# getzlab/rnaseqc

Hardware: AMD Instinct MI355X
Metric: reads/sec whole-node (100 M-read synthetic BAM, GENCODE GTF) at 1/2/4/8 GPU -- `value`: the hot path over the records resident in HBM (the bench contract's definition of value); `whole_node.value`: the same job from the BAM file to the reports (CLI `Average Reads/Sec` window), checked against `value (higher is better)
Workload: dtype i32/u64 counters, f64 exon fractions

## Files before the change

rnaseqc_amd/csrc/rsqc_api.cpp:

```cpp
#include "rsqc_ctx.h"
#include "rsqc_index.h"

namespace rsqc {

int fail(rsqc_ctx *c, int code, const std::string &msg) {
    if (c) { c->last_error = msg; }
    return code;
}
int dev_alloc(rsqc_ctx *c, DevBuf &b, size_t bytes, bool zero) {
    if (bytes == 0) bytes = 16;
    bytes = (bytes + 15) & ~(size_t)15;
    if (b.bytes < bytes) {
        b.release();
        HIP_TRY(c, hipMalloc(&b.p, bytes));
        b.bytes = bytes;
    }
    if (zero) HIP_TRY(c, hipMemsetAsync(b.p, 0, b.bytes, c->stream));
    return 0;
}

static int zero_accumulators(rsqc_ctx *c) {
    launch_reset(c->stream, c->d_arena.p, c->arena_bytes, c->d_cov.p, c->d_cov.bytes, (uint32_t *)((char *)c->d_arena.p + c->off_misc + 36));
    HIP_TRY(c, hipGetLastError());
    for (auto &pb : c->pair_pool) pb.used = false;
    c->pairs_in_flight.clear();
    c->pair_arena.used = c->frag_arena.used = c->gc_arena.used = 0;
    for (auto &fb : c->frag_pool) fb.used = false;
    c->frags_in_flight.clear();
    c->h_fsize.clear(); c->h_fcount.clear();
    c->frag_remaining = c->have_bed ? c->params.fragment_samples : 0;
    for (auto &gb : c->gc_pool) gb.used = false;
    c->gcs_in_flight.clear();
    if (c->have_ref) {
        HIP_TRY(c, hipMemsetAsync(c->d_gc_bins.p, 0, (RSQC_GC_BINS + 1) * 8, c->stream));
        c->h_gc.assign(RSQC_GC_BINS + 1, 0);
    }
    c->finalized = false;
// ... 27 lines not shown
        delete c;
        return RSQC_ERR_HIP;
    }
    c->dparams.mapq_threshold = params->mapq_threshold;
    c->dparams.base_mismatch = params->base_mismatch;
    c->dparams.chimeric_distance = params->chimeric_distance;
    c->dparams.stranded = params->stranded;
    c->dparams.unpaired = params->unpaired;
    c->dparams.exclude_chimeric = params->exclude_chimeric;
    c->dparams.n_filter_tags = params->n_filter_tags;
    c->dparams.legacy = params->legacy ? 1 : 0;
    c->pair_arena.n_col = 1; c->pair_arena.width[0] = sizeof(PairRec);
    c->frag_arena.n_col = 6; { const size_t w[6] = {8, 8, 4, 4, 4, 4}; for (int k = 0; k < 6; ++k) c->frag_arena.width[k] = w[k]; }
    c->gc_arena.n_col = 7; { const size_t w[7] = {8, 8, 4, 4, 4, 4, 4}; for (int k = 0; k < 7; ++k) c->gc_arena.width[k] = w[k]; }
    if (const char *e = getenv("RSQC_K1_GRID")) c->k1_grid = std::min(16384, std::max(1, atoi(e)));
    *out = c;
    return RSQC_OK;
}

void rsqc_destroy(rsqc_ctx *c) {
    if (!c) return;
    (void)hipSetDevice(c->device);
    (void)hipStreamSynchronize(c->stream);
    for (auto *u : c->resident) if (u) free_batch(u);
    for (auto *u : c->transient) free_batch(u);
    for (auto &b : c->upload_pool) b.release();
    for (auto &b : c->ann_bufs) b.release();
    for (auto &pb : c->pair_pool) { pb.rec.release(); pb.counts.release(); if (pb.h_counts) (void)hipHostFree(pb.h_counts); if (pb.done) (void)hipEventDestroy(pb.done); if (pb.kernels) (void)hipEventDestroy(pb.kernels); }
    for (auto &fb : c->frag_pool) { fb.file.release(); fb.qhash.release(); fb.name.release(); fb.endpos.release(); fb.fs.release(); fb.h2.release(); fb.count.release(); fb.r_file.release(); fb.r_qhash.release(); fb.r_name.release(); fb.r_endpos.release(); fb.r_fs.release(); fb.r_h2.release(); fb.r_counts.release(); if (fb.h_count) (void)hipHostFree(fb.h_count); }
    for (auto &gb : c->gc_pool) { gb.file.release(); gb.qhash.release(); gb.row.release(); gb.endpos.release(); gb.flag_lq.release(); gb.tid.release(); gb.h2.release(); gb.count.release(); if (gb.h_count) (void)hipHostFree(gb.h_count); }
// ... 15 lines not shown
    track_drop(c, true);
    for (auto &b : c->parked) b.release();
    free_sort_scratch(c->gc_scratch); free_sort_scratch(c->frag_scratch);
    c->d_ref_bits.release(); c->d_ref_off.release(); c->d_ref_len.release(); c->d_gc_bins.release(); c->d_exon_gc.release();
    DevBuf *all[] = {&c->d_arena, &c->d_cov, &c->d_ovf_index, &c->d_tiles, &c->d_defer, &c->d_ei_rank, &c->d_table, &c->d_tab_off, &c->d_tab_cap};
    if (c->h_arena) (void)hipHostFree(c->h_arena);
    if (c->h_rl_raw) (void)hipHostFree(c->h_rl_raw);
    if (c->stream2) (void)hipStreamDestroy(c->stream2);
    if (c->stream3) (void)hipStreamDestroy(c->stream3);
    if (c->stream4) (void)hipStreamDestroy(c->stream4);
    if (c->ev_join3) (void)hipEventDestroy(c->ev_join3);
    if (c->ev_join4) (void)hipEventDestroy(c->ev_join4);
    if (c->ev_fork) (void)hipEventDestroy(c->ev_fork);
    if (c->ev_retired) (void)hipEventDestroy(c->ev_retired);
    if (c->ev_join) (void)hipEventDestroy(c->ev_join);
    for (auto *b : all) b->release();
    for (auto &pr : c->k1_events) { (void)hipEventDestroy(pr.first); (void)hipEventDestroy(pr.second); }
    for (auto &pr : c->long_events) (void)hipEventDestroy(pr.second);
    for (auto e : c->event_pool) (void)hipEventDestroy(e);
    (void)hipStreamDestroy(c->stream);
    delete c;
}

int rsqc_set_annotation(rsqc_ctx *c, const rsqc_annotation *a, const uint8_t *owned_contig) {
    if (!c || !a) return RSQC_ERR_ARG;
    if (c->have_ann) return fail(c, RSQC_ERR_ARG, "annotation already set");
    HIP_TRY(c, hipSetDevice(c->device));
    const int nc = a->n_contigs, G = a->n_genes, L = a->n_genes_listed, E = a->n_exons;
    c->n_ref = a->n_ref; c->n_contigs = nc; c->n_genes = G; c->n_listed = L; c->n_exons = E;
    HostIndex hx;
// ... 65 lines not shown
    c->off_gcv = at; at += Lz * 8;
    c->off_ecv = at; at += Ez * 8;
    c->off_gvalid = at; at += pad8(Lz);
    c->off_ecvv = at; at += pad8(Ez);
    c->off_ehit = at; at += pad8(Ez);
    at = (at + 15) & ~(size_t)15;
    c->off_misc = at; at += 64;
    c->arena_bytes = at;
    if ((rc = dev_alloc(c, c->d_arena, at, false))) return rc;
    HIP_TRY(c, hipHostMalloc((void **)&c->h_arena, at, hipHostMallocDefault));
    if ((rc = dev_alloc(c, c->d_cov, (size_t)(run + 64) * 4, false))) return rc;
    const uint32_t ovf_cap = 1u << 20;
    if ((rc = dev_alloc(c, c->d_ovf_index, (size_t)ovf_cap * 8, false))) return rc;
    for (hipStream_t *s : {&c->stream2, &c->stream3, &c->stream4})
        if (!*s) HIP_TRY(c, hipStreamCreateWithPriority(s, hipStreamNonBlocking, c->prio_side));
    for (hipEvent_t *e : {&c->ev_join3, &c->ev_join4, &c->ev_fork, &c->ev_join, &c->ev_retired})
        if (!*e) HIP_TRY(c, hipEventCreateWithFlags(e, hipEventDisableTiming));
    char *A = (char *)c->d_arena.p;
    DevAccum &acc = c->acc;
    acc.gene_reads = (unsigned long long *)(A + c->off_u64);
    acc.gene_unique = acc.gene_reads + G;
    acc.gene_frag = acc.gene_unique + G;
    acc.counters = acc.gene_frag + G;
    acc.exon_acc = (double *)(A + c->off_exon);
    acc.cov_diff = (uint32_t *)c->d_cov.p;
    acc.ovf_count = (uint32_t *)(A + c->off_misc);
    acc.read_length = (int32_t *)(A + c->off_misc + 8);
    acc.error = (int *)(A + c->off_misc + 16);
    acc.rl_stats = (uint32_t *)(A + c->off_misc + 32);
    acc.defer_total = (uint32_t *)(A + c->off_misc + 48);
    acc.ovf_index = (uint64_t *)c->d_ovf_index.p; acc.ovf_cap = ovf_cap;
    c->have_ann = true;
    if ((rc = zero_accumulators(c))) return rc;
    HIP_TRY(c, hipStreamSynchronize(c->stream));
    c->last_error = hx.warning;
    c->n_exons_outside_gene = hx.n_exons_outside_gene;
    return RSQC_OK;
}

int rsqc_set_reference(rsqc_ctx *c, const rsqc_reference *ref) {
    if (!c || !ref || !c->have_ann) return RSQC_ERR_ARG;
    if (c->have_ref) return fail(c, RSQC_ERR_ARG, "reference already set");
    HIP_TRY(c, hipSetDevice(c->device));
    const int nc = c->n_contigs;
    std::vector<unsigned long long> off((size_t)nc, ~0ull), len((size_t)nc, 0ull);
    unsigned long long words = 0, longest = 0;
    for (int i = 0; i < ref->n; ++i) {
// ... 124 lines not shown
    c->arena_bytes = 0;
    c->dann = DevAnnotation{}; c->dref = DevReference{};
    uint32_t *const tile_span = c->acc.tile_span;
    c->acc = DevAccum{}; c->acc.tile_span = tile_span;
    c->d_ge_off = c->d_ge_row = c->d_gene_cov_off = c->d_gene_coding = c->d_gene_order = nullptr;
    c->d_gene_flags = c->d_gene_owned = nullptr;
    c->n_ref = c->n_contigs = c->n_genes = c->n_listed = c->n_exons = 0;
    c->k3_large = c->k3_medium = c->k3_xlarge = c->k3_le6144 = c->k3_le3072 = c->k3_le2048 = c->k3_le1024 = 0;
    c->cov_entries = 0; c->n_exons_outside_gene = 0;
    std::vector<uint32_t>().swap(c->exon_row_id);
    std::vector<double>().swap(c->h_exon_gc);
    c->h_gc.clear();
    c->have_ann = c->have_bed = c->have_ref = false;
    free_sort_scratch(c->gc_scratch); free_sort_scratch(c->frag_scratch);
    c->h_fsize.clear(); c->h_fcount.clear(); c->frag_remaining = 0; c->frag_kept = 0;
    c->finalized = false; c->early_copied = false;
    c->next_record_base = 0; c->name_mode = -1; c->have_ranges = false; c->have_composed_rl = false;
    c->batch_file_index.clear(); c->batch_records.clear();
    c->h_rl_offset.clear(); c->h_rl_span.clear(); c->h_rl_state.clear();
    c->h_sample_file.clear(); c->h_sample_size.clear();
    c->results = rsqc_results{};
    c->sticky = 0;
    c->last_error.clear();
    return RSQC_OK;
}

void *rsqc_host_alloc(size_t bytes) {
    void *p = nullptr;
    if (hipHostMalloc(&p, bytes ? bytes : 16, hipHostMallocDefault) != hipSuccess) { (void)hipGetLastError(); return nullptr; }
    return p;
}
// ... 49 lines not shown
```

rnaseqc_amd/csrc/rsqc_ctx.h:

```cpp
#pragma once
#include <algorithm>
#include <chrono>
#include <cstdio>
#include <cstdlib>
#include <cstring>
#include <string>
#include <vector>

#include "rsqc_device.h"
#include "rsqc_decode.h"
#include "rsqc_sam.h"

#if defined(RSQC_K1_PROF) || defined(RSQC_DIAG_KNOBS)
#define RSQC_DIAG(name) getenv(name)
namespace rsqc {
inline void host_trace(const char *what) {
    static const bool on = getenv("RSQC_HOST_TRACE") != nullptr;
    if (!on) return;
    static std::chrono::steady_clock::time_point last = std::chrono::steady_clock::now();
    const auto now = std::chrono::steady_clock::now();
    fprintf(stderr, "[host] %-28s +%8.1f us\n", what, std::chrono::duration<double, std::micro>(now - last).count());
    last = now;
}
}
// ... 145 lines not shown
    uint32_t k3_large = 0, k3_medium = 0, k3_xlarge = 0, k3_le6144 = 0, k3_le3072 = 0, k3_le2048 = 0, k3_le1024 = 0;
    int stream_prio = 0, prio_side = 0;
    uint32_t n_exons_outside_gene = 0;
    hipEvent_t fin_e0 = nullptr, fin_e1 = nullptr;
    uint64_t cov_entries = 0;
    bool have_bed = false;

    DevBuf d_arena, d_cov, d_ovf_index, d_tiles;
    DevBuf d_defer;
    DevBuf d_ei_rank;
    char *h_arena = nullptr;
    size_t arena_bytes = 0, off_u64 = 0, off_exon = 0, off_gmean = 0, off_gstd = 0, off_gcv = 0, off_bias3 = 0,
           off_bias5 = 0, off_ecv = 0, off_gvalid = 0, off_ecvv = 0, off_ehit = 0, off_misc = 0;
    hipStream_t stream2 = nullptr, stream3 = nullptr, stream4 = nullptr;
    hipEvent_t ev_fork = nullptr, ev_join = nullptr, ev_join3 = nullptr, ev_join4 = nullptr, ev_retired = nullptr;
    DevAccum acc{};
    uint64_t tile_cap = 0;
    std::vector<PairBuf> pair_pool;
    std::vector<size_t> pairs_in_flight;
    Arena pair_arena, frag_arena, gc_arena;
    DevBuf d_arena_count;
    std::vector<DevBuf> parked;
    DevBuf d_table, d_tab_off, d_tab_cap;
    std::vector<FragBuf> frag_pool;
    std::vector<size_t> frags_in_flight;
    uint32_t frag_remaining = 0;
    bool have_ref = false;
    DevBuf d_ref_bits, d_ref_off, d_ref_len, d_gc_bins, d_exon_gc;
    DevReference dref{};
    std::vector<GcBuf> gc_pool;
    std::vector<size_t> gcs_in_flight;
    std::vector<uint64_t> h_gc;
    std::vector<double> h_exon_gc;
    SortScratch gc_scratch, frag_scratch;
    uint32_t frag_kept = 0;
    bool finalized = false;

    std::vector<UploadedBatch *> resident;
// ... 75 lines not shown
```

rnaseqc_amd/csrc/rsqc_device.h:

```cpp
#pragma once

#if !defined(RSQC_WAVE_EMU)
#include <hip/hip_runtime.h>
#endif
#include <stdint.h>

#include "rsqc_read.h"

#define RSQC_K1_THREADS 256
#define RSQC_MAX_BIAS_WINDOW 1024
#define RSQC_K3_THREADS 1024
#include "rsqc_k3_plan.h"

namespace rsqc {

struct DevBatch {
    uint64_t n;
    uint64_t record_base;
    const rsqc_rec_core *core;
    const rsqc_rec_aux *aux;
    const uint32_t *cigar;
    const uint32_t *qhash2;
    uint32_t n_seg;
    const int32_t *seg_tid;
// ... 86 lines not shown
    const unsigned long long *gene_reads;
    uint32_t *cov;
    int32_t n_listed;
    uint32_t mask; int32_t bias_offset, bias_window; uint64_t bias_gene_length;
    double *g_mean, *g_std, *g_cv; uint8_t *g_valid;
    double *e_cv; uint8_t *e_cv_valid;
    unsigned long long *bias3, *bias5;
    int *error;
};
void launch_gene_coverage(hipStream_t s, hipStream_t s2, hipStream_t s3, const GeneCovArgs &A, uint32_t n_large, uint32_t n_medium, uint32_t n_xlarge,
                          uint32_t n_le6144 = 0, uint32_t n_le3072 = 0, uint32_t n_le2048 = 0, uint32_t n_le1024 = 0);

void launch_reduce_add(hipStream_t s, unsigned long long *du, const unsigned long long *su, size_t nu, double *df, const double *sf, size_t nf,
                       uint8_t *db, const uint8_t *sb, size_t nb);
void launch_pack_results(hipStream_t s, const double *exon_acc, uint8_t *exon_hit, uint32_t n_exons);
void launch_reset(hipStream_t s, void *arena, size_t arena_bytes, void *cov, size_t cov_bytes, uint32_t *rl_min);
void launch_classify(hipStream_t s, int grid, int variant, const DevAnnotation &a, const DevParams &p, const DevBatch &b,
                     const DevAccum &acc);
inline int rsqc_long_grid(int k1_grid) { return k1_grid < 1024 ? k1_grid : 1024; }
void launch_classify_long(hipStream_t s, int k1_grid, const DevAnnotation &a, const DevParams &p, const DevBatch &b, const DevAccum &acc);
void launch_ei_rank(hipStream_t s, const EiEntry *ei, uint32_t ei_lo, uint32_t ei_hi, EiRank *rank, uint32_t n_words);
void launch_classify_slow(hipStream_t s, const DevAnnotation &a, const DevParams &p, const DevBatch &b,
                          const DevAccum &acc);
#define RSQC_RL_SUMMARY_WORDS (2 + 2 * 128)
void launch_read_length(hipStream_t s, const DevAnnotation &a, const DevParams &p, const DevBatch &b,
                        const DevAccum &acc, uint32_t *summary);
#define RSQC_SLOW_RES 2048u
#define RSQC_SLOW_LEGACY_GRID 4096u
#ifndef RSQC_K4_PART_READS
#define RSQC_K4_PART_READS 1024
#endif
#define RSQC_K4_SUB_CAP (2 * RSQC_K4_PART_READS)
#define RSQC_K4_PART_SLOTS (4 * RSQC_K4_PART_READS)
#ifndef RSQC_K4_COUNT_THREADS
#define RSQC_K4_COUNT_THREADS 256
#endif
struct FragKey { uint32_t lo, hi, h2; };
struct FragPlan {
    uint32_t *part_first;
    uint32_t *cursor;
    uint4 *ginfo;
    uint4 *part_info;
    uint32_t *full_list, *full_n;
    FragKey *list;
    unsigned long long *blk_space; uint32_t *blk_parts;
};
void launch_frag_layout(hipStream_t s, const unsigned long long *gene_reads, uint32_t n_genes, const FragPlan &P, int *error);
void launch_frag_local(hipStream_t s, const DevAccum &acc, uint32_t n_chunks, const FragPlan &P, uint32_t list_blocks);
void launch_pairs_append(hipStream_t s, const PairRec *src, uint32_t chunk_cap, const uint32_t *counts,
                         uint32_t n_chunks, uint32_t slow_base, uint32_t slow_cap, PairRec *dst);
void launch_frag_count(hipStream_t s, uint32_t n_genes, const FragPlan &P, uint32_t parts_bound, unsigned long long *gene_frag, int *error);

}

#include <vector>
namespace rsqc {
struct SortScratch { void *k0 = nullptr, *k1 = nullptr, *v0 = nullptr, *v1 = nullptr, *v2 = nullptr, *v3 = nullptr, *tmp = nullptr, *count = nullptr;
                     size_t cap_n = 0, tmp_bytes = 0; uint32_t *table = nullptr, *out_size = nullptr, *out_count = nullptr; };
void free_sort_scratch(SortScratch &s);
int run_fragment_sizes(hipStream_t stream, const FragCandidates &c, uint32_t n, uint32_t max_samples,
                       std::vector<int64_t> &sizes, std::vector<uint64_t> &counts, uint32_t &remaining, SortScratch &S, uint32_t &n_kept, int *d_error);
void launch_frag_compact(hipStream_t s, const FragCandidates &src, const FragCandidates &dst, uint64_t n_rec, int k1_grid);
void launch_gc_pack(hipStream_t s, const uint8_t *ascii, uint64_t len, unsigned long long *words);
void launch_exon_gc(hipStream_t s, const DevAnnotation &a, const DevReference &R, double *exon_gc);
void launch_gc_candidates(hipStream_t s, const DevAnnotation &a, const DevParams &p, const DevBatch &b, const DevReference &R,
                          const GcCandidates &out, int *error);
// ... 3 lines not shown
```

rnaseqc_amd/csrc/rsqc_finalize.cpp:

```cpp
#include "rsqc_ctx.h"

static int read_back(rsqc_ctx *c) {
    const int G = c->n_genes, L = c->n_listed, E = c->n_exons;
    char *A = (char *)c->d_arena.p;
    if (c->early_copied) {
        const size_t frag_lo = c->off_u64 + (size_t)2 * (size_t)G * 8;
        HIP_TRY(c, hipMemcpyAsync(c->h_arena + frag_lo, (char *)c->d_arena.p + frag_lo, (size_t)G * 8, hipMemcpyDeviceToHost, c->stream));
        HIP_TRY(c, hipMemcpyAsync(c->h_arena + c->off_misc, (char *)c->d_arena.p + c->off_misc, c->arena_bytes - c->off_misc, hipMemcpyDeviceToHost, c->stream));
        c->early_copied = false;
        RSQC_TRACE("read_back: copies enqueued");
    } else {
        launch_pack_results(c->stream, (const double *)(A + c->off_exon), (uint8_t *)(A + c->off_ehit), (uint32_t)E);
        HIP_TRY(c, hipMemcpyAsync(c->h_arena, c->d_arena.p, c->arena_bytes, hipMemcpyDeviceToHost, c->stream));
    }
    HIP_TRY(c, hipStreamSynchronize(c->stream));
    RSQC_TRACE("read_back: stream idle");
    char *H = c->h_arena;
    uint64_t *u = (uint64_t *)(H + c->off_u64);
    rsqc_results &R = c->results;
    for (int k = 0; k < RSQC_N_COUNTERS; ++k) R.counters[k] = u[3 * (size_t)G + (size_t)k];
    R.n_genes_listed = L; R.n_exons = E;
    R.gene_reads = u; R.gene_unique = u + G; R.gene_fragments = u + 2 * (size_t)G;
    R.exon_reads = (double *)(H + c->off_exon); R.exon_hit = (uint8_t *)(H + c->off_ehit);
    R.read_length = c->have_composed_rl ? c->composed_rl : *(const int32_t *)(H + c->off_misc + 8);
// ... 82 lines not shown
                acc.pairs = (PairRec *)c->pair_arena.col[0].p;
                acc.pair_chunk_cap = 0; acc.pair_chunk_count = (uint32_t *)c->d_arena_count.p;
                acc.pair_slow_base = 0; acc.pair_slow_cap = used32;
                launch_frag_local(c->stream, acc, 0, P, (uint32_t)std::min<uint64_t>(4096, c->pair_arena.used / 1024 + 1));
            }
            for (size_t idx : c->pairs_in_flight) {
                if (RSQC_DIAG("RSQC_DIAG_SKIP_K4")) break;
                PairBuf &pb = c->pair_pool[idx];
                DevAccum acc = c->acc;
                acc.pairs = (PairRec *)pb.rec.p;
                acc.pair_chunk_cap = pb.chunk_cap; acc.pair_chunk_count = (uint32_t *)pb.counts.p;
                acc.pair_slow_base = pb.slow_base; acc.pair_slow_cap = pb.slow_cap;
                acc.pair_slow_count = (uint32_t *)pb.counts.p + pb.n_chunks;
                launch_frag_local(c->stream, acc, pb.n_chunks, P, c->dparams.legacy ? (uint32_t)std::min<uint64_t>(4096, pb.slow_cap / 8192 + 32) : 0u);
            }
            if (!RSQC_DIAG("RSQC_DIAG_SKIP_K4")) launch_frag_count(c->stream, (uint32_t)G, P, (uint32_t)parts_bound, c->acc.gene_frag, c->acc.error);
        }
        RSQC_TRACE("finalize: K3 + K4 enqueued");
        {
            const size_t nb = c->batch_file_index.size();
            if (nb * RSQC_RL_SUMMARY_WORDS > c->h_rl_raw_cap) {
                if (c->h_rl_raw) { (void)hipHostFree(c->h_rl_raw); c->h_rl_raw = nullptr; c->h_rl_raw_cap = 0; }
                const size_t want = std::max<size_t>(2 * nb, 64) * RSQC_RL_SUMMARY_WORDS;
                HIP_TRY(c, hipHostMalloc((void **)&c->h_rl_raw, want * 4, hipHostMallocDefault));
                c->h_rl_raw_cap = want;
            }
            RSQC_TRACE("finalize: K3 enqueued");
            if (nb) HIP_TRY(c, hipMemcpyAsync(c->h_rl_raw, c->d_rl_summary.p, nb * RSQC_RL_SUMMARY_WORDS * 4, hipMemcpyDeviceToHost, c->stream2));
            RSQC_TRACE("finalize: rl copy call returned");
        }
        HIP_TRY(c, hipEventRecord(c->ev_join3, c->stream3));
        HIP_TRY(c, hipEventRecord(c->ev_join4, c->stream4));
        if (early_readback) {
            const size_t frag_lo = c->off_u64 + (size_t)2 * (size_t)c->n_genes * 8, frag_hi = frag_lo + (size_t)c->n_genes * 8;
            HIP_TRY(c, hipStreamWaitEvent(c->stream2, c->ev_join3, 0));
            HIP_TRY(c, hipStreamWaitEvent(c->stream2, c->ev_join4, 0));
            launch_pack_results(c->stream2, (const double *)(A + c->off_exon), (uint8_t *)(A + c->off_ehit), (uint32_t)c->n_exons);
            if (frag_lo) HIP_TRY(c, hipMemcpyAsync(c->h_arena, c->d_arena.p, frag_lo, hipMemcpyDeviceToHost, c->stream2));
            HIP_TRY(c, hipMemcpyAsync(c->h_arena + frag_hi, (char *)c->d_arena.p + frag_hi, c->off_misc - frag_hi, hipMemcpyDeviceToHost, c->stream2));
            c->early_copied = true;
        }
        HIP_TRY(c, hipEventRecord(c->ev_join, c->stream2));
        HIP_TRY(c, hipStreamWaitEvent(c->stream, c->ev_join, 0));
        HIP_TRY(c, hipStreamWaitEvent(c->stream, c->ev_join3, 0));
        HIP_TRY(c, hipStreamWaitEvent(c->stream, c->ev_join4, 0));
        HIP_TRY(c, hipGetLastError());
        HIP_TRY(c, hipEventRecord(e1, c->stream));
        if (c->have_bed) {
            uint64_t incoming = 0;
            bool beside = true;
#ifdef RSQC_K5_SERIAL
            beside = false;
#endif
            HIP_TRY(c, hipEventSynchronize(c->ev_fork));
            for (size_t k = 0; k < c->frags_in_flight.size(); ++k) incoming += *c->frag_pool[c->frags_in_flight[k]].h_count;
            if (c->frag_arena.used && c->frag_arena.used + incoming > c->frag_arena.cap) beside = false;
            hipStream_t ks = beside ? c->stream4 : c->stream;
            if (!beside) HIP_TRY(c, hipStreamSynchronize(c->stream));
            else if (retired_here) HIP_TRY(c, hipStreamWaitEvent(ks, c->ev_retired, 0));
            for (size_t k = 0; k < c->frags_in_flight.size(); ++k) {
// ... 177 lines not shown
```

rnaseqc_amd/csrc/rsqc_k4.h:

```cpp
#pragma once

namespace rsqc {


__device__ __forceinline__ uint32_t frag_part_hash(uint64_t key) {
    uint32_t h = (uint32_t)(key >> 32);
    h ^= h >> 15; h *= 0x2C1B3C6Du; h ^= h >> 12;
    return h;
}
__device__ __forceinline__ uint32_t frag_parts_of(unsigned long long reads) {
    return (uint32_t)((reads + RSQC_K4_PART_READS - 1) / RSQC_K4_PART_READS);
}
__device__ __forceinline__ uint32_t frag_cap_of(unsigned long long reads) {
    return frag_parts_of(reads) == 1 ? (uint32_t)reads : (uint32_t)RSQC_K4_SUB_CAP;
}
__device__ __forceinline__ unsigned long long frag_space_of(unsigned long long reads) {
    return ((unsigned long long)frag_parts_of(reads) * frag_cap_of(reads) + 15ull) & ~15ull;
}
__global__ void __launch_bounds__(1024)
frag_layout_totals_kernel(const unsigned long long *gene_reads, uint32_t n_genes, unsigned long long *blk_space, uint32_t *blk_parts, int *error) {
    __shared__ unsigned long long w_space[16];
    __shared__ uint32_t w_parts[16];
    const uint32_t g = blockIdx.x * 1024u + threadIdx.x;
    unsigned long long space = 0; uint32_t parts = 0;
// ... 208 lines not shown
        }
        RSQC_FIN_SECT(32, 6);
#ifdef RSQC_K1_PROF
        if (threadIdx.x == 0) atomicAdd(&g_fin_prof[32 + 15], 1ull);
#endif
#pragma unroll
        for (int u = 0; u < U; ++u) { g[u] = gn[u]; key[u] = keyn[u]; h2[u] = h2n[u]; }
    }
}

template <int SLOTS>
__global__ void __launch_bounds__(RSQC_K4_COUNT_THREADS)
frag_count_kernel(const uint32_t *n_parts_at, const uint32_t *cursor, const uint4 *part_info, const FragKey *list,
                  unsigned long long *gene_frag, uint32_t *full_list, uint32_t *full_n, int *error) {
    constexpr bool LISTED = SLOTS == RSQC_K4_PART_SLOTS;
    __shared__ unsigned long long s_keys[SLOTS];
    __shared__ uint32_t s_h2[SLOTS];
    constexpr uint32_t OVF = 32;
    __shared__ unsigned long long s_ovk[OVF];
    __shared__ uint32_t s_ov2[OVF], s_ovn;
    __shared__ uint32_t s_fresh[2];
    constexpr int KPT = (SLOTS / 2) / RSQC_K4_COUNT_THREADS;
    constexpr uint32_t N_LO = SLOTS == RSQC_K4_PART_SLOTS ? (uint32_t)SLOTS / 4u : 0u;
    const uint32_t n_parts = LISTED ? *full_n : *n_parts_at;
    struct Row { uint32_t fill; uint4 info; bool fuller; };
    auto row_of = [&](uint32_t i) -> Row {
        Row r; r.fill = 0u; r.info = make_uint4(0u, 0u, 0u, 0u); r.fuller = false;
        if (i < n_parts) {
            const uint32_t w = LISTED ? full_list[i] : i;
            r.fill = cursor[w]; r.info = part_info[w];
            const uint32_t n = r.fill < r.info.y ? r.fill : r.info.y;
            r.fuller = n > (uint32_t)SLOTS / 2u;
// ... 38 lines not shown
#if defined(__HIP_DEVICE_COMPILE__)
#define K4_UNI(x) ((uint32_t)__builtin_amdgcn_readfirstlane((int)(x)))
#else
#define K4_UNI(x) ((uint32_t)(x))
#endif
    RSQC_FIN_BEGIN
    while (w < n_parts) {
        RSQC_FIN_SECT(48, 0);
        const Row nn = row_of(w + 2u * gridDim.x);
        keys_of(nxt, kvn, k2n);
        if (!LISTED && cur.fuller && threadIdx.x == 0) full_list[atomicAdd(full_n, 1u)] = w;
        if (cur.fill != 0u) {
            const uint32_t gene = K4_UNI(cur.info.x), cap = K4_UNI(cur.info.y), fill = K4_UNI(cur.fill);
            const uint32_t n = fill < cap ? fill : cap;
            uint32_t slots = 64;
            while (slots < 2 * n && slots < (uint32_t)SLOTS) slots <<= 1;
            const uint32_t smask = slots - 1;
            for (uint32_t i = threadIdx.x; i < slots; i += blockDim.x) s_keys[i] = 0ull;
            __syncthreads();
            if (owe && threadIdx.x == 0) settle();
            RSQC_FIN_SECT(48, 1);
            uint32_t fresh = 0;
            constexpr uint32_t NO_SLOT = 0xFFFFFFFFu;
            auto insert = [&](unsigned long long k, uint32_t h2) -> uint32_t {
                uint32_t slot = (((uint32_t)k * 0x9E3779B1u) >> 16) & smask;
#pragma unroll 1
                for (uint32_t probe = 0; probe < slots; ++probe) {
                    const unsigned long long old = atomicCAS(&s_keys[slot], 0ull, k);
                    if (old == 0ull) { s_h2[slot] = h2; ++fresh; return NO_SLOT; }
                    if (old == k) return slot;
                    slot = (slot + 1) & smask;
                }
                atomicExch(error, RSQC_ERR_CAPACITY);
                return NO_SLOT;
            };
            uint32_t same[KPT];
#pragma unroll
            for (int j = 0; j < KPT; ++j) same[j] = ((uint32_t)j * RSQC_K4_COUNT_THREADS + threadIdx.x < n) ? insert(kv[j], k2[j]) : NO_SLOT;
            static_assert(RSQC_K4_SUB_CAP <= RSQC_K4_PART_SLOTS / 2 && RSQC_K4_PART_READS <= RSQC_K4_PART_SLOTS / 2, "a list fits the registers of its instance");
            if (n > (uint32_t)KPT * RSQC_K4_COUNT_THREADS) atomicExch(error, RSQC_ERR_CAPACITY);
            __syncthreads();
#pragma unroll
            for (int j = 0; j < KPT; ++j)
                if (same[j] != NO_SLOT && s_h2[same[j]] != k2[j]) {
                    const uint32_t at = atomicAdd(&s_ovn, 1u);
                    if (at < OVF) { s_ovk[at] = kv[j]; s_ov2[at] = k2[j]; } else atomicExch(error, RSQC_ERR_CAPACITY);
// ... 24 lines not shown
```

rnaseqc_amd/csrc/rsqc_kernels.hip:

```cpp
#include <hip/hip_runtime.h>
#include <stdint.h>
#include <algorithm>
#include <cstdlib>

#ifdef RSQC_K1_PROF
namespace rsqc { __device__ __forceinline__ void k1_mark(int sec); __device__ __forceinline__ void k1_event(int id, bool cond); }
#define RSQC_MARK(sec) ::rsqc::k1_mark(sec)
#define RSQC_EVENT(id, cond) ::rsqc::k1_event(id, cond)
#endif

#include "rsqc_device.h"
#ifndef RSQC_K1_PROF
#define RSQC_FIN_STAMP(sec)
#define RSQC_FIN_SECT(base, sec)
#define RSQC_FIN_BEGIN
#endif

namespace rsqc {

}
#include "rsqc_wave.h"
namespace rsqc {

#ifdef RSQC_K1_PROF
// ... 274 lines not shown
reduce_add_kernel(unsigned long long *du, const unsigned long long *su, size_t nu, double *df, const double *sf, size_t nf,
                  uint8_t *db, const uint8_t *sb, size_t nb) {
    const size_t stride = (size_t)gridDim.x * blockDim.x, t = (size_t)blockIdx.x * blockDim.x + threadIdx.x;
    for (size_t i = t; i < nu; i += stride) du[i] += su[i];
    for (size_t i = t; i < nf; i += stride) df[i] += sf[i];
    for (size_t i = t; i < nb; i += stride) db[i] = (uint8_t)(db[i] + sb[i]);
}
void launch_reduce_add(hipStream_t s, unsigned long long *du, const unsigned long long *su, size_t nu, double *df, const double *sf, size_t nf,
                       uint8_t *db, const uint8_t *sb, size_t nb) {
    hipLaunchKernelGGL(reduce_add_kernel, dim3(512), dim3(256), 0, s, du, su, nu, df, sf, nf, db, sb, nb);
}

void launch_pack_results(hipStream_t s, const double *exon_acc, uint8_t *exon_hit, uint32_t n_exons) {
    if (n_exons) hipLaunchKernelGGL(pack_results_kernel, dim3((n_exons + 255) / 256 < 1024 ? (n_exons + 255) / 256 : 1024), dim3(256), 0, s, exon_acc, exon_hit, n_exons);
}
void launch_reset(hipStream_t s, void *arena, size_t arena_bytes, void *cov, size_t cov_bytes, uint32_t *rl_min) {
    const size_t rl_vec = (size_t)((char *)rl_min - 4 - (char *)arena) / 16;
    hipLaunchKernelGGL(reset_kernel, dim3(1024), dim3(256), 0, s, (uint4 *)arena, (arena_bytes + 15) / 16, (uint4 *)cov, (cov_bytes + 15) / 16, rl_vec);
}
void launch_frag_compact(hipStream_t s, const FragCandidates &src, const FragCandidates &dst, uint64_t n_rec, int k1_grid) {
    hipLaunchKernelGGL(frag_compact_kernel, dim3(k1_grid), dim3(256), 0, s, src, dst, (uint32_t)n_rec, (uint32_t)k1_grid);
}
void launch_classify(hipStream_t s, int grid, int variant, const DevAnnotation &a, const DevParams &p, const DevBatch &b,
                     const DevAccum &acc) {
    if (variant < 0) hipLaunchKernelGGL(classify_count_kernel_legacy, dim3(grid), dim3(RSQC_K1_THREADS), 0, s, a, p, b, acc);
    else {
#if defined(RSQC_K1_PROF) || defined(RSQC_DIAG_KNOBS)
        static const unsigned pad = getenv("RSQC_K1_LDS_PAD") ? (unsigned)atoi(getenv("RSQC_K1_LDS_PAD")) : 0u;
#else
        const unsigned pad = 0u;
#endif
        const K1Args A{a, p, b, acc};
        if (a.have_bed) hipLaunchKernelGGL(classify_ei_kernel<true>, dim3(grid), dim3(RSQC_K1_THREADS), pad, s, A);
// ... 17 lines not shown
void launch_read_length(hipStream_t s, const DevAnnotation &a, const DevParams &p, const DevBatch &b,
                        const DevAccum &acc, uint32_t *summary) {
    hipLaunchKernelGGL(read_length_kernel, dim3(acc.rl_seg ? b.n_seg : 1u), dim3(64), 0, s, a, p, b, acc, summary);
}
void launch_frag_layout(hipStream_t s, const unsigned long long *gene_reads, uint32_t n_genes, const FragPlan &P, int *error) {
    const uint32_t blocks = (n_genes + 1023u) / 1024u;
    if (!blocks) return;
    hipLaunchKernelGGL(frag_layout_totals_kernel, dim3(blocks), dim3(1024), 0, s, gene_reads, n_genes, P.blk_space, P.blk_parts, error);
    hipLaunchKernelGGL(frag_layout_kernel, dim3(blocks), dim3(1024), 0, s, gene_reads, n_genes, P.blk_space, P.blk_parts, P.part_first,
                       P.ginfo, P.cursor, P.part_info, P.full_n);
}
void launch_frag_local(hipStream_t s, const DevAccum &acc, uint32_t n_chunks, const FragPlan &P, uint32_t list_blocks) {
    hipLaunchKernelGGL(frag_local_kernel, dim3(frag_local_chunk_wgs(n_chunks) + (list_blocks ? list_blocks : RSQC_K4_SLOW_BLOCKS)), dim3(RSQC_K4L_THREADS), 0, s, acc.pairs, acc.pair_chunk_cap, acc.pair_chunk_count, n_chunks, acc.pair_slow_base, acc.pair_slow_cap,
                       P.ginfo, P.cursor, P.list, acc.error);
}
void launch_frag_count(hipStream_t s, uint32_t n_genes, const FragPlan &P, uint32_t parts_bound, unsigned long long *gene_frag, int *error) {
    if (n_genes == 0) return;
    const uint32_t grid = parts_bound < 16384u ? (parts_bound ? parts_bound : 1u) : 16384u;
    hipLaunchKernelGGL((frag_count_kernel<RSQC_K4_PART_SLOTS / 2>), dim3(grid), dim3(RSQC_K4_COUNT_THREADS), 0, s, P.part_first + n_genes, P.cursor, P.part_info, P.list, gene_frag,
                       P.full_list, P.full_n, error);
    hipLaunchKernelGGL((frag_count_kernel<RSQC_K4_PART_SLOTS>), dim3(grid < 1024u ? grid : 1024u), dim3(RSQC_K4_COUNT_THREADS), 0, s, P.part_first + n_genes, P.cursor, P.part_info, P.list, gene_frag,
                       P.full_list, P.full_n, error);
}
#ifndef RSQC_K3_MEDIUM_T
#define RSQC_K3_MEDIUM_T uint32_t
#endif
#ifndef RSQC_K3_SMALL_T
#define RSQC_K3_SMALL_T uint32_t
#endif
void launch_gene_coverage(hipStream_t s, hipStream_t s2, hipStream_t s3, const GeneCovArgs &A, uint32_t n_large, uint32_t n_medium, uint32_t n_xlarge,
                          uint32_t n_le6144, uint32_t n_le3072, uint32_t n_le2048, uint32_t n_le1024) {
    if (A.n_listed <= 0) return;
    K3Launch plan[RSQC_K3_LAUNCHES];
    k3_plan((uint32_t)A.n_listed, n_large, n_medium, n_xlarge, n_le6144, n_le3072, n_le2048, n_le1024, plan);
    const hipStream_t streams[3] = {s, s2, s3};
    const bool wide = A.bias_window > 128;
// ... 25 lines not shown
```

rnaseqc_amd/csrc/rsqc_submit.cpp:

```cpp
#include "rsqc_ctx.h"

namespace rsqc {

const char *device_error_text(int err) {
    return err == RSQC_ERR_BAD_CIGAR ? "Unrecognized Cigar Op" :
           err == RSQC_ERR_CAPACITY ? "a device-side capacity was exceeded" :
           err == RSQC_ERR_EMPTY_MEDIAN ? "Cannot compute median of an empty list" : "device error";
}
hipEvent_t get_event(rsqc_ctx *c) {
    if (!c->event_pool.empty()) { hipEvent_t e = c->event_pool.back(); c->event_pool.pop_back(); return e; }
    hipEvent_t e = nullptr;
    (void)hipEventCreate(&e);
    return e;
}
int resolve_events(rsqc_ctx *c) {
    auto add = [&](std::vector<std::pair<hipEvent_t, hipEvent_t>> &events, auto &total, bool recycle_first) {
        for (auto &pr : events) {
            float ms = 0.f;
            if (hipEventElapsedTime(&ms, pr.first, pr.second) == hipSuccess) total += ms;
            if (recycle_first) c->event_pool.push_back(pr.first);
            c->event_pool.push_back(pr.second);
        }
        events.clear();
    };
// ... 187 lines not shown
        c->gc_pool.push_back(gb);
    }
    GcBuf &gb = c->gc_pool[gidx];
    gb.used = true;
    c->gcs_in_flight.push_back(gidx);
    HIP_TRY(c, hipMemsetAsync(gb.count.p, 0, 16, c->stream));
    *out = &gb;
    return 0;
}

int run_batch(rsqc_ctx *c, UploadedBatch *u) {
    if (u->n >= (1ull << 31)) return fail(c, RSQC_ERR_ARG, "batch too large (split it)");
    if (!c->have_ann) return fail(c, RSQC_ERR_ARG, "rsqc_set_annotation must precede rsqc_submit");
    if (c->finalized) return fail(c, RSQC_ERR_ARG, "rsqc_reset required after rsqc_finalize");
    if (u->n == 0) return 0;
    {
        const int mode = u->d.qhash2 ? 1 : 0;
        if (c->name_mode < 0) c->name_mode = mode;
        else if (c->name_mode != mode)
            return fail(c, RSQC_ERR_ARG, "rsqc_batch.qhash2 must be given for every batch of a pass or for none (the name identity is 96 or 64 bits for the whole pass)");
    }
    if (c->sort.active) return sort_append(c, u);
    const uint64_t tiles = (u->n + RSQC_K1_THREADS - 1) / RSQC_K1_THREADS;
    const uint64_t wave_tiles = (u->n + 63) / 64 + 64;
    if (wave_tiles > c->tile_cap) {
        c->tile_cap = wave_tiles + wave_tiles / 4 + 64;
        int rc = dev_alloc(c, c->d_tiles, c->tile_cap * sizeof(uint32_t), false);
        if (rc) return rc;
        c->acc.tile_span = (uint32_t *)c->d_tiles.p;
    }
// ... 165 lines not shown
```

Measured before the change: 26.58 billion.

## Zero coverage buffer during finalize on a side stream; size K4 grids by occupancy

Finalize now clears the coverage buffer on stream3 after its last consumers finish, so the following reset can skip that memset while the buffer is known clean. The frag_count kernel grids are sized from the device's CU count times the occupancy-reported resident blocks instead of fixed caps. The small-partition hash table is enlarged to a non-power-of-two set, using multiply-shift range reduction for wide partitions. This adds state tracking (cov_clean) and extra cross-stream waits, which risks stale coverage if the invariant is broken.

New measurement: 26.69 billion (median of 6 runs). No clear change (+0.4%).

```diff
diff --git a/rnaseqc_amd/csrc/rsqc_api.cpp b/rnaseqc_amd/csrc/rsqc_api.cpp
--- a/rnaseqc_amd/csrc/rsqc_api.cpp
+++ b/rnaseqc_amd/csrc/rsqc_api.cpp
@@ -20,7 +20,8 @@
 }
 
 static int zero_accumulators(rsqc_ctx *c) {
-    launch_reset(c->stream, c->d_arena.p, c->arena_bytes, c->d_cov.p, c->d_cov.bytes, (uint32_t *)((char *)c->d_arena.p + c->off_misc + 36));
+    const bool cov_is_zero = c->cov_clean && c->finalized && !c->sticky;
+    launch_reset(c->stream, c->d_arena.p, c->arena_bytes, c->d_cov.p, cov_is_zero ? 0 : c->d_cov.bytes, (uint32_t *)((char *)c->d_arena.p + c->off_misc + 36));
     HIP_TRY(c, hipGetLastError());
     for (auto &pb : c->pair_pool) pb.used = false;
     c->pairs_in_flight.clear();
@@ -78,6 +79,7 @@
     c->frag_arena.n_col = 6; { const size_t w[6] = {8, 8, 4, 4, 4, 4}; for (int k = 0; k < 6; ++k) c->frag_arena.width[k] = w[k]; }
     c->gc_arena.n_col = 7; { const size_t w[7] = {8, 8, 4, 4, 4, 4, 4}; for (int k = 0; k < 7; ++k) c->gc_arena.width[k] = w[k]; }
     if (const char *e = getenv("RSQC_K1_GRID")) c->k1_grid = std::min(16384, std::max(1, atoi(e)));
+    if (frag_count_resident(&c->k4_resident)) { rsqc_destroy(c); return RSQC_ERR_HIP; }
     *out = c;
     return RSQC_OK;
 }
@@ -123,6 +125,8 @@
     if (c->ev_fork) (void)hipEventDestroy(c->ev_fork);
     if (c->ev_retired) (void)hipEventDestroy(c->ev_retired);
     if (c->ev_join) (void)hipEventDestroy(c->ev_join);
+    if (c->ev_cov2) (void)hipEventDestroy(c->ev_cov2);
+    if (c->ev_clean) (void)hipEventDestroy(c->ev_clean);
     for (auto *b : all) b->release();
     for (auto &pr : c->k1_events) { (void)hipEventDestroy(pr.first); (void)hipEventDestroy(pr.second); }
     for (auto &pr : c->long_events) (void)hipEventDestroy(pr.second);
@@ -218,7 +222,7 @@
     if ((rc = dev_alloc(c, c->d_ovf_index, (size_t)ovf_cap * 8, false))) return rc;
     for (hipStream_t *s : {&c->stream2, &c->stream3, &c->stream4})
         if (!*s) HIP_TRY(c, hipStreamCreateWithPriority(s, hipStreamNonBlocking, c->prio_side));
-    for (hipEvent_t *e : {&c->ev_join3, &c->ev_join4, &c->ev_fork, &c->ev_join, &c->ev_retired})
+    for (hipEvent_t *e : {&c->ev_join3, &c->ev_join4, &c->ev_fork, &c->ev_join, &c->ev_retired, &c->ev_cov2, &c->ev_clean})
         if (!*e) HIP_TRY(c, hipEventCreateWithFlags(e, hipEventDisableTiming));
     char *A = (char *)c->d_arena.p;
     DevAccum &acc = c->acc;
@@ -235,6 +239,7 @@
     acc.defer_total = (uint32_t *)(A + c->off_misc + 48);
     acc.ovf_index = (uint64_t *)c->d_ovf_index.p; acc.ovf_cap = ovf_cap;
     c->have_ann = true;
+    c->cov_clean = false;
     if ((rc = zero_accumulators(c))) return rc;
     HIP_TRY(c, hipStreamSynchronize(c->stream));
     c->last_error = hx.warning;
@@ -389,7 +394,7 @@
     c->have_ann = c->have_bed = c->have_ref = false;
     free_sort_scratch(c->gc_scratch); free_sort_scratch(c->frag_scratch);
     c->h_fsize.clear(); c->h_fcount.clear(); c->frag_remaining = 0; c->frag_kept = 0;
-    c->finalized = false; c->early_copied = false;
+    c->finalized = false; c->early_copied = false; c->cov_clean = false;
     c->next_record_base = 0; c->name_mode = -1; c->have_ranges = false; c->have_composed_rl = false;
     c->batch_file_index.clear(); c->batch_records.clear();
     c->h_rl_offset.clear(); c->h_rl_span.clear(); c->h_rl_state.clear();
diff --git a/rnaseqc_amd/csrc/rsqc_ctx.h b/rnaseqc_amd/csrc/rsqc_ctx.h
--- a/rnaseqc_amd/csrc/rsqc_ctx.h
+++ b/rnaseqc_amd/csrc/rsqc_ctx.h
@@ -183,6 +183,7 @@
            off_bias5 = 0, off_ecv = 0, off_gvalid = 0, off_ecvv = 0, off_ehit = 0, off_misc = 0;
     hipStream_t stream2 = nullptr, stream3 = nullptr, stream4 = nullptr;
     hipEvent_t ev_fork = nullptr, ev_join = nullptr, ev_join3 = nullptr, ev_join4 = nullptr, ev_retired = nullptr;
+    hipEvent_t ev_cov2 = nullptr, ev_clean = nullptr;
     DevAccum acc{};
     uint64_t tile_cap = 0;
     std::vector<PairBuf> pair_pool;
@@ -191,6 +192,8 @@
     DevBuf d_arena_count;
     std::vector<DevBuf> parked;
     DevBuf d_table, d_tab_off, d_tab_cap;
+    FragCountGrid k4_resident{};
+    bool cov_clean = false;
     std::vector<FragBuf> frag_pool;
     std::vector<size_t> frags_in_flight;
     uint32_t frag_remaining = 0;
diff --git a/rnaseqc_amd/csrc/rsqc_device.h b/rnaseqc_amd/csrc/rsqc_device.h
--- a/rnaseqc_amd/csrc/rsqc_device.h
+++ b/rnaseqc_amd/csrc/rsqc_device.h
@@ -124,7 +124,10 @@
 void launch_reduce_add(hipStream_t s, unsigned long long *du, const unsigned long long *su, size_t nu, double *df, const double *sf, size_t nf,
                        uint8_t *db, const uint8_t *sb, size_t nb);
 void launch_pack_results(hipStream_t s, const double *exon_acc, uint8_t *exon_hit, uint32_t n_exons);
-void launch_reset(hipStream_t s, void *arena, size_t arena_bytes, void *cov, size_t cov_bytes, uint32_t *rl_min);
+#ifndef RSQC_COV_ZERO_BLOCKS
+#define RSQC_COV_ZERO_BLOCKS 64
+#endif
+void launch_reset(hipStream_t s, void *arena, size_t arena_bytes, void *cov, size_t cov_bytes, uint32_t *rl_min, uint32_t blocks = 1024);
 void launch_classify(hipStream_t s, int grid, int variant, const DevAnnotation &a, const DevParams &p, const DevBatch &b,
                      const DevAccum &acc);
 inline int rsqc_long_grid(int k1_grid) { return k1_grid < 1024 ? k1_grid : 1024; }
@@ -145,6 +148,12 @@
 #ifndef RSQC_K4_COUNT_THREADS
 #define RSQC_K4_COUNT_THREADS 256
 #endif
+#ifndef RSQC_K4_SMALL_SET
+#define RSQC_K4_SMALL_SET 1664
+#endif
+#ifndef RSQC_K4_COUNT_ROUNDS
+#define RSQC_K4_COUNT_ROUNDS 8
+#endif
 struct FragKey { uint32_t lo, hi, h2; };
 struct FragPlan {
     uint32_t *part_first;
@@ -159,7 +168,9 @@
 void launch_frag_local(hipStream_t s, const DevAccum &acc, uint32_t n_chunks, const FragPlan &P, uint32_t list_blocks);
 void launch_pairs_append(hipStream_t s, const PairRec *src, uint32_t chunk_cap, const uint32_t *counts,
                          uint32_t n_chunks, uint32_t slow_base, uint32_t slow_cap, PairRec *dst);
-void launch_frag_count(hipStream_t s, uint32_t n_genes, const FragPlan &P, uint32_t parts_bound, unsigned long long *gene_frag, int *error);
+struct FragCountGrid { uint32_t small_wgs, large_wgs; };
+int frag_count_resident(FragCountGrid *out);
+void launch_frag_count(hipStream_t s, uint32_t n_genes, const FragPlan &P, uint32_t parts_bound, const FragCountGrid &resident, unsigned long long *gene_frag, int *error);
 
 }
 
diff --git a/rnaseqc_amd/csrc/rsqc_finalize.cpp b/rnaseqc_amd/csrc/rsqc_finalize.cpp
--- a/rnaseqc_amd/csrc/rsqc_finalize.cpp
+++ b/rnaseqc_amd/csrc/rsqc_finalize.cpp
@@ -120,7 +120,7 @@
                 acc.pair_slow_count = (uint32_t *)pb.counts.p + pb.n_chunks;
                 launch_frag_local(c->stream, acc, pb.n_chunks, P, c->dparams.legacy ? (uint32_t)std::min<uint64_t>(4096, pb.slow_cap / 8192 + 32) : 0u);
             }
-            if (!RSQC_DIAG("RSQC_DIAG_SKIP_K4")) launch_frag_count(c->stream, (uint32_t)G, P, (uint32_t)parts_bound, c->acc.gene_frag, c->acc.error);
+            if (!RSQC_DIAG("RSQC_DIAG_SKIP_K4")) launch_frag_count(c->stream, (uint32_t)G, P, (uint32_t)parts_bound, c->k4_resident, c->acc.gene_frag, c->acc.error);
         }
         RSQC_TRACE("finalize: K3 + K4 enqueued");
         {
@@ -137,6 +137,7 @@
         }
         HIP_TRY(c, hipEventRecord(c->ev_join3, c->stream3));
         HIP_TRY(c, hipEventRecord(c->ev_join4, c->stream4));
+        HIP_TRY(c, hipEventRecord(c->ev_cov2, c->stream2));
         if (early_readback) {
             const size_t frag_lo = c->off_u64 + (size_t)2 * (size_t)c->n_genes * 8, frag_hi = frag_lo + (size_t)c->n_genes * 8;
             HIP_TRY(c, hipStreamWaitEvent(c->stream2, c->ev_join3, 0));
@@ -146,10 +147,17 @@
             HIP_TRY(c, hipMemcpyAsync(c->h_arena + frag_hi, (char *)c->d_arena.p + frag_hi, c->off_misc - frag_hi, hipMemcpyDeviceToHost, c->stream2));
             c->early_copied = true;
         }
+        HIP_TRY(c, hipStreamWaitEvent(c->stream3, c->ev_cov2, 0));
+        HIP_TRY(c, hipStreamWaitEvent(c->stream3, c->ev_join4, 0));
+        launch_reset(c->stream3, c->d_arena.p, 0, c->d_cov.p, c->d_cov.bytes, (uint32_t *)((char *)c->d_arena.p + c->off_misc + 36), RSQC_COV_ZERO_BLOCKS);
+        HIP_TRY(c, hipGetLastError());
+        HIP_TRY(c, hipEventRecord(c->ev_clean, c->stream3));
         HIP_TRY(c, hipEventRecord(c->ev_join, c->stream2));
         HIP_TRY(c, hipStreamWaitEvent(c->stream, c->ev_join, 0));
         HIP_TRY(c, hipStreamWaitEvent(c->stream, c->ev_join3, 0));
         HIP_TRY(c, hipStreamWaitEvent(c->stream, c->ev_join4, 0));
+        HIP_TRY(c, hipStreamWaitEvent(c->stream, c->ev_clean, 0));
+        c->cov_clean = true;
         HIP_TRY(c, hipGetLastError());
         HIP_TRY(c, hipEventRecord(e1, c->stream));
         if (c->have_bed) {
diff --git a/rnaseqc_amd/csrc/rsqc_k4.h b/rnaseqc_amd/csrc/rsqc_k4.h
--- a/rnaseqc_amd/csrc/rsqc_k4.h
+++ b/rnaseqc_amd/csrc/rsqc_k4.h
@@ -246,8 +246,11 @@
 frag_count_kernel(const uint32_t *n_parts_at, const uint32_t *cursor, const uint4 *part_info, const FragKey *list,
                   unsigned long long *gene_frag, uint32_t *full_list, uint32_t *full_n, int *error) {
     constexpr bool LISTED = SLOTS == RSQC_K4_PART_SLOTS;
-    __shared__ unsigned long long s_keys[SLOTS];
-    __shared__ uint32_t s_h2[SLOTS];
+    constexpr uint32_t SET = LISTED ? (uint32_t)SLOTS : (uint32_t)RSQC_K4_SMALL_SET;
+    constexpr uint32_t POW2_TOP = LISTED ? (uint32_t)SLOTS : (uint32_t)SLOTS / 2u;
+    static_assert(SET > (uint32_t)SLOTS / 2u && SET >= POW2_TOP && SET % 64u == 0u && SET < 65536u, "every key of the fullest partition finds a slot; the range reduction takes 16 bits");
+    __shared__ unsigned long long s_keys[SET];
+    __shared__ uint32_t s_h2[SET];
     constexpr uint32_t OVF = 32;
     __shared__ unsigned long long s_ovk[OVF];
     __shared__ uint32_t s_ov2[OVF], s_ovn;
@@ -316,7 +319,9 @@
             const uint32_t gene = K4_UNI(cur.info.x), cap = K4_UNI(cur.info.y), fill = K4_UNI(cur.fill);
             const uint32_t n = fill < cap ? fill : cap;
             uint32_t slots = 64;
-            while (slots < 2 * n && slots < (uint32_t)SLOTS) slots <<= 1;
+            while (slots < 2 * n && slots < POW2_TOP) slots <<= 1;
+            const bool wide = 2 * n > POW2_TOP;
+            if (wide) slots = SET;
             const uint32_t smask = slots - 1;
             for (uint32_t i = threadIdx.x; i < slots; i += blockDim.x) s_keys[i] = 0ull;
             __syncthreads();
@@ -325,13 +330,14 @@
             uint32_t fresh = 0;
             constexpr uint32_t NO_SLOT = 0xFFFFFFFFu;
             auto insert = [&](unsigned long long k, uint32_t h2) -> uint32_t {
-                uint32_t slot = (((uint32_t)k * 0x9E3779B1u) >> 16) & smask;
+                const uint32_t hh = ((uint32_t)k * 0x9E3779B1u) >> 16;
+                uint32_t slot = wide ? (hh * SET) >> 16 : hh & smask;
 #pragma unroll 1
                 for (uint32_t probe = 0; probe < slots; ++probe) {
                     const unsigned long long old = atomicCAS(&s_keys[slot], 0ull, k);
                     if (old == 0ull) { s_h2[slot] = h2; ++fresh; return NO_SLOT; }
                     if (old == k) return slot;
-                    slot = (slot + 1) & smask;
+                    slot = slot + 1 == slots ? 0u : slot + 1;
                 }
                 atomicExch(error, RSQC_ERR_CAPACITY);
                 return NO_SLOT;
diff --git a/rnaseqc_amd/csrc/rsqc_kernels.hip b/rnaseqc_amd/csrc/rsqc_kernels.hip
--- a/rnaseqc_amd/csrc/rsqc_kernels.hip
+++ b/rnaseqc_amd/csrc/rsqc_kernels.hip
@@ -312,9 +312,9 @@
 void launch_pack_results(hipStream_t s, const double *exon_acc, uint8_t *exon_hit, uint32_t n_exons) {
     if (n_exons) hipLaunchKernelGGL(pack_results_kernel, dim3((n_exons + 255) / 256 < 1024 ? (n_exons + 255) / 256 : 1024), dim3(256), 0, s, exon_acc, exon_hit, n_exons);
 }
-void launch_reset(hipStream_t s, void *arena, size_t arena_bytes, void *cov, size_t cov_bytes, uint32_t *rl_min) {
+void launch_reset(hipStream_t s, void *arena, size_t arena_bytes, void *cov, size_t cov_bytes, uint32_t *rl_min, uint32_t blocks) {
     const size_t rl_vec = (size_t)((char *)rl_min - 4 - (char *)arena) / 16;
-    hipLaunchKernelGGL(reset_kernel, dim3(1024), dim3(256), 0, s, (uint4 *)arena, (arena_bytes + 15) / 16, (uint4 *)cov, (cov_bytes + 15) / 16, rl_vec);
+    hipLaunchKernelGGL(reset_kernel, dim3(blocks ? blocks : 1u), dim3(256), 0, s, (uint4 *)arena, (arena_bytes + 15) / 16, (uint4 *)cov, (cov_bytes + 15) / 16, rl_vec);
 }
 void launch_frag_compact(hipStream_t s, const FragCandidates &src, const FragCandidates &dst, uint64_t n_rec, int k1_grid) {
     hipLaunchKernelGGL(frag_compact_kernel, dim3(k1_grid), dim3(256), 0, s, src, dst, (uint32_t)n_rec, (uint32_t)k1_grid);
@@ -362,12 +362,22 @@
     hipLaunchKernelGGL(frag_local_kernel, dim3(frag_local_chunk_wgs(n_chunks) + (list_blocks ? list_blocks : RSQC_K4_SLOW_BLOCKS)), dim3(RSQC_K4L_THREADS), 0, s, acc.pairs, acc.pair_chunk_cap, acc.pair_chunk_count, n_chunks, acc.pair_slow_base, acc.pair_slow_cap,
                        P.ginfo, P.cursor, P.list, acc.error);
 }
-void launch_frag_count(hipStream_t s, uint32_t n_genes, const FragPlan &P, uint32_t parts_bound, unsigned long long *gene_frag, int *error) {
+int frag_count_resident(FragCountGrid *out) {
+    int dev = 0, cus = 0, small = 0, large = 0;
+    if (hipGetDevice(&dev) != hipSuccess || hipDeviceGetAttribute(&cus, hipDeviceAttributeMultiprocessorCount, dev) != hipSuccess) return 1;
+    if (hipOccupancyMaxActiveBlocksPerMultiprocessor(&small, frag_count_kernel<RSQC_K4_PART_SLOTS / 2>, RSQC_K4_COUNT_THREADS, 0) != hipSuccess ||
+        hipOccupancyMaxActiveBlocksPerMultiprocessor(&large, frag_count_kernel<RSQC_K4_PART_SLOTS>, RSQC_K4_COUNT_THREADS, 0) != hipSuccess) return 1;
+    if (cus <= 0 || small <= 0 || large <= 0) return 1;
+    out->small_wgs = (uint32_t)cus * (uint32_t)small; out->large_wgs = (uint32_t)cus * (uint32_t)large;
+    return 0;
+}
+void launch_frag_count(hipStream_t s, uint32_t n_genes, const FragPlan &P, uint32_t parts_bound, const FragCountGrid &resident, unsigned long long *gene_frag, int *error) {
     if (n_genes == 0) return;
-    const uint32_t grid = parts_bound < 16384u ? (parts_bound ? parts_bound : 1u) : 16384u;
-    hipLaunchKernelGGL((frag_count_kernel<RSQC_K4_PART_SLOTS / 2>), dim3(grid), dim3(RSQC_K4_COUNT_THREADS), 0, s, P.part_first + n_genes, P.cursor, P.part_info, P.list, gene_frag,
+    const uint32_t parts = parts_bound ? parts_bound : 1u;
+    const uint32_t small = resident.small_wgs * RSQC_K4_COUNT_ROUNDS, large = resident.large_wgs;
+    hipLaunchKernelGGL((frag_count_kernel<RSQC_K4_PART_SLOTS / 2>), dim3(parts < small ? parts : small), dim3(RSQC_K4_COUNT_THREADS), 0, s, P.part_first + n_genes, P.cursor, P.part_info, P.list, gene_frag,
                        P.full_list, P.full_n, error);
-    hipLaunchKernelGGL((frag_count_kernel<RSQC_K4_PART_SLOTS>), dim3(grid < 1024u ? grid : 1024u), dim3(RSQC_K4_COUNT_THREADS), 0, s, P.part_first + n_genes, P.cursor, P.part_info, P.list, gene_frag,
+    hipLaunchKernelGGL((frag_count_kernel<RSQC_K4_PART_SLOTS>), dim3(parts < large ? parts : large), dim3(RSQC_K4_COUNT_THREADS), 0, s, P.part_first + n_genes, P.cursor, P.part_info, P.list, gene_frag,
                        P.full_list, P.full_n, error);
 }
 #ifndef RSQC_K3_MEDIUM_T
diff --git a/rnaseqc_amd/csrc/rsqc_submit.cpp b/rnaseqc_amd/csrc/rsqc_submit.cpp
--- a/rnaseqc_amd/csrc/rsqc_submit.cpp
+++ b/rnaseqc_amd/csrc/rsqc_submit.cpp
@@ -225,6 +225,7 @@
     if (!c->have_ann) return fail(c, RSQC_ERR_ARG, "rsqc_set_annotation must precede rsqc_submit");
     if (c->finalized) return fail(c, RSQC_ERR_ARG, "rsqc_reset required after rsqc_finalize");
     if (u->n == 0) return 0;
+    c->cov_clean = false;
     {
         const int mode = u->d.qhash2 ? 1 : 0;
         if (c->name_mode < 0) c->name_mode = mode;
```
